# xxxupeng/stereo_toolbox

Measured on AMD Instinct MI355X. Metric: stereo pairs/sec @ 540x960 D=192 (GwcNet_GC fwd+bwd), higher is better.
Workload: dtype f32; 1 GPU; GwcNet_GC(maxdisp=192) train step: fwd+bwd+allreduce+Adam, 576x960 pairs (reference pad_to_2x shape), batch 1/GPU, fp32, synthetic randn inputs, deterministic filler weights; global_batch=1, parallelism=dp1, grad_sync=none (single rank: flat fp32 buffer packed, no collective), launch=eager, optimizer=torch.optim.Adam(fused=True)

## Files before the change

stereo_toolbox_amd/csrc/conv3d.hip:

```cpp
#include "stx_common.h"
#include <stdlib.h>

namespace {

constexpr int CONV_THREADS = 256;

struct ConvArgs {
    const float* x;
    const float* wp;
    float* out;
    const float* scale;
    const float* bias;
    const float* residual;
    float* stats;
    int Di, Hi, Wi, Cin;
    int Do, Ho, Wo, Cout;
    int relu;
    int nDt, nHt, nWt;
};

__device__ __forceinline__ int xcd_remap(int bid, int nblk) {
    const int q = nblk >> 3, r = nblk & 7;
    const int xcd = bid & 7, k = bid >> 3;
    const int base = (xcd < r) ? xcd * (q + 1) : r * (q + 1) + (xcd - r) * q;
// ... 873 lines not shown
    const float* f;
    const float* c;
    float* slab;
    int B, Df, Hf, Wf, CF;
    int Dc, Hc, Wc, CC;
    int nHt, nWt, ntiles;
    int ablate;
};

template <int KS, int S, int TH, int TW, int NW, bool PIPE>
__global__ __launch_bounds__(NW * 64) void conv3d_wgrad_kernel(WgradArgs a) {
    constexpr int NTHR = NW * 64;
    constexpr int PAD = KS / 2;
    constexpr int T = KS * KS * KS;
    constexpr int ED = KS, EH = (TH - 1) * S + KS, EW = (TW - 1) * S + KS;
    constexpr int EWH = (EW + 1) / 2;
    constexpr int EWS = (S == 2) ? 2 * EWH : EW;
    constexpr int NTAP = (T + NW - 1) / NW;
    constexpr int NV = TH * TW;
    STX_DYN_SMEM(smem);
    float* ftile = reinterpret_cast<float*>(smem);
    float* ctile = ftile + ED * EH * EWS * 32;

    const int tid = threadIdx.x, lane = tid & 63;
    const int wave = __builtin_amdgcn_readfirstlane(tid >> 6);
    const int i = lane & 31, half = lane >> 5;
    const int ncf = a.CF / 32;
    const int cfb = blockIdx.y % ncf, ccb = blockIdx.y / ncf;

    f32x16 acc[NTAP];
#pragma unroll
    for (int t = 0; t < NTAP; ++t) acc[t] = zero16();

    constexpr int NPL = (EH * EW * 8 + NTHR - 1) / NTHR;
    constexpr int NFL = ED * NPL;
    constexpr int NCL = (NV * 8 + NTHR - 1) / NTHR;
    float4 sf[NFL], sc[NCL];
    unsigned fbase[NPL], cbase[NCL];
    int fhw[NPL], chw[NCL];
#pragma unroll
    for (int k = 0; k < NPL; ++k) {
        const int idx = tid + k * NTHR;
        const int v = idx >> 3, f = idx & 7;
        const int wx = v % EW, hy = v / EW;
        fhw[k] = idx < EH * EW * 8 ? (hy << 16 | wx) : -1;
        fbase[k] = (unsigned)(((hy * a.Wf + wx) * a.CF + cfb * 32 + 4 * f) * 4);
    }
#pragma unroll
    for (int k = 0; k < NCL; ++k) {
        const int idx = tid + k * NTHR;
        const int v = idx >> 3, f = idx & 7;
        chw[k] = idx < NV * 8 ? ((v / TW) << 16 | (v % TW)) : -1;
        cbase[k] = (unsigned)((((v / TW) * a.Wc + v % TW) * a.CC + ccb * 32 + 4 * f) * 4);
    }
    const long long fplane = (long long)a.Hf * a.Wf, cplane = (long long)a.Hc * a.Wc;
    auto load_tile = [&](int tile, bool on) {
        int r = tile;
        const int wt = r % a.nWt; r /= a.nWt;
        const int ht = r % a.nHt; r /= a.nHt;
        const int od = r % a.Dc;
        const int b = r / a.Dc;
        const int oh0 = ht * TH, ow0 = wt * TW;
        const int id0 = od * S - PAD, ih0 = oh0 * S - PAD, iw0 = ow0 * S - PAD;
        unsigned fvo[NPL];
#pragma unroll
        for (int k = 0; k < NPL; ++k) {
            const int gh = ih0 + (fhw[k] >> 16), gw = iw0 + (fhw[k] & 0xffff);
            fvo[k] = (fhw[k] >= 0 && gh >= 0 && gh < a.Hf && gw >= 0 && gw < a.Wf) ? fbase[k] : STX_BUF_OOB;
        }
        const long long forg = (long long)ih0 * a.Wf + iw0;
#pragma unroll
        for (int dz = 0; dz < ED; ++dz) {
            const int gd = id0 + dz;
            const bool in = on && gd >= 0 && gd < a.Df;
            const stx_bufrsrc rs = stx_make_rsrc(a.f + (((long long)b * a.Df + (in ? gd : 0)) * fplane + forg) * a.CF,
                                                 in ? (unsigned)((fplane - forg) * a.CF * 4) : 0u);
#pragma unroll
            for (int k = 0; k < NPL; ++k) sf[dz * NPL + k] = stx_buf_ld4(rs, fvo[k], 0u);
        }
        const long long corg = (long long)oh0 * a.Wc + ow0;
        const stx_bufrsrc rc = stx_make_rsrc(a.c + (((long long)b * a.Dc + od) * cplane + corg) * a.CC,
                                             on ? (unsigned)((cplane - corg) * a.CC * 4) : 0u);
#pragma unroll
        for (int k = 0; k < NCL; ++k) {
            const bool ok = chw[k] >= 0 && oh0 + (chw[k] >> 16) < a.Hc && ow0 + (chw[k] & 0xffff) < a.Wc;
            sc[k] = stx_buf_ld4(rc, ok ? cbase[k] : STX_BUF_OOB, 0u);
        }
    };
    auto store_tile = [&]() {
#pragma unroll
        for (int dz = 0; dz < ED; ++dz)
#pragma unroll
            for (int k = 0; k < NPL; ++k) {
                const int wx = fhw[k] & 0xffff, hy = fhw[k] >> 16;
                const int slot = (S == 2) ? (wx & 1) * EWH + (wx >> 1) : wx;
                const int f = (tid + k * NTHR) & 7;
                if (fhw[k] >= 0) stx_st4(ftile + ((dz * EH + hy) * EWS + slot) * 32 + 4 * f, sf[dz * NPL + k]);
            }
#pragma unroll
        for (int k = 0; k < NCL; ++k) {
            const int idx = tid + k * NTHR;
            if (idx < NV * 8) stx_st4(ctile + (idx >> 3) * 32 + 4 * (idx & 7), sc[k]);
        }
    };

    if (PIPE && (int)blockIdx.x < a.ntiles) load_tile(blockIdx.x, a.ablate != 1);
    for (int tile = blockIdx.x; tile < a.ntiles; tile += gridDim.x) {
        if (!PIPE) load_tile(tile, a.ablate != 1);
        __syncthreads();
        if (a.ablate != 1) store_tile();
        __syncthreads();
        if (PIPE) {
            const int nxt = tile + (int)gridDim.x;
            load_tile(nxt < a.ntiles ? nxt : tile, nxt < a.ntiles && a.ablate != 1);
        }
        if (a.ablate == 2) continue;
        if (KS == 1) {
            for (int p = wave; p < NV / 2; p += NW) {
                const int v = 2 * p + half;
                const int lw = v % TW, lh = v / TW;
                const float bv = ctile[v * 32 + i];
                const float av = ftile[(lh * EWS + lw) * 32 + i];
                acc[0] = __builtin_amdgcn_mfma_f32_32x32x2f32(av, bv, acc[0], 0, 0, 0);
            }
        } else {
            int toff[NTAP];
#pragma unroll
            for (int t = 0; t < NTAP; ++t) {
                const int tap = (t * NW + wave < T) ? t * NW + wave : 0;
                const int kd = tap / 9, kh = (tap / 3) % 3, kw = tap % 3;
                toff[t] = (S == 2) ? ((kd * EH + kh) * EWS + (kw & 1) * EWH + (kw >> 1)) * 32
                                   : ((kd * EH + kh) * EWS + kw) * 32;
            }
            float av[2][NTAP], bv[2];
            auto load_pair = [&](int p, int buf) {
                const int v = 2 * p + half;
                const int lw = v % TW, lh = v / TW;
                const int vb = ((lh * S) * EWS + lw) * 32 + i;
                bv[buf] = ctile[v * 32 + i];
#pragma unroll
                for (int t = 0; t < NTAP; ++t) av[buf][t] = ftile[vb + toff[t]];
            };
            auto mma_pair = [&](int buf) {
#pragma unroll
                for (int t = 0; t < NTAP; ++t)
                    if (t * NW + wave < T) acc[t] = __builtin_amdgcn_mfma_f32_32x32x2f32(av[buf][t], bv[buf], acc[t], 0, 0, 0);
            };
            load_pair(0, 0);
            for (int p = 0; p < NV / 2; p += 2) {
                load_pair(p + 1, 1);
                STX_SCHED_BARRIER();
                mma_pair(0);
                STX_SCHED_BARRIER();
                load_pair((p + 2 < NV / 2) ? p + 2 : 0, 0);
                STX_SCHED_BARRIER();
                mma_pair(1);
                STX_SCHED_BARRIER();
            }
        }
    }
    constexpr int ROWS = (KS == 1) ? NW : T;
    float* dst = a.slab + ((size_t)blockIdx.y * gridDim.x + blockIdx.x) * ROWS * 1024;
#pragma unroll
    for (int t = 0; t < NTAP; ++t) {
        const int row = (KS == 1) ? wave : t * NW + wave;
        if (KS == 1 ? (t == 0) : (row < T)) {
#pragma unroll
            for (int r = 0; r < 16; ++r) {
                const int cf = (r & 3) + 8 * (r >> 2) + 4 * half;
                dst[(size_t)row * 1024 + cf * 32 + i] = acc[t][r];
            }
        }
    }
}

__global__ __launch_bounds__(CONV_THREADS) void conv3d_wgrad_reduce4_kernel(const float* __restrict__ slab,
                                                                            float* __restrict__ dw, int CF, int CC,
                                                                            int T, int nchunks, int rows_per_chunk) {
    __shared__ float red[16][64];
    const int lane = threadIdx.x & 63, wave = threadIdx.x >> 6;
    const int part = wave * 4 + (lane >> 4), ql = lane & 15;
    const int idx0 = blockIdx.x * 64 + ql * 4;
    const int cc_l = idx0 & 31, cf_l = (idx0 >> 5) & 31;
    const int tap = (idx0 >> 10) % T, pair = (idx0 >> 10) / T;
    const float* p;
    size_t stride;
    int n;
    if (rows_per_chunk == T) {
        p = slab + ((size_t)pair * nchunks * T + tap) * 1024 + cf_l * 32 + cc_l;
        stride = (size_t)T * 1024; n = nchunks;
    } else {
        p = slab + ((size_t)pair * nchunks * rows_per_chunk) * 1024 + cf_l * 32 + cc_l;
        stride = 1024; n = nchunks * rows_per_chunk;
    }
    float4 s = make_float4(0.f, 0.f, 0.f, 0.f);
#pragma unroll 4
    for (int c = part; c < n; c += 16) {
        const float4 v = stx_ld4(p + (size_t)c * stride);
        s.x += v.x; s.y += v.y; s.z += v.z; s.w += v.w;
    }
    stx_st4(&red[part][ql * 4], s);
    __syncthreads();
    if (wave == 0) {
        float t = 0.f;
#pragma unroll
        for (int k = 0; k < 16; ++k) t += red[k][lane];
        const int idx = blockIdx.x * 64 + lane;
        const int cc = idx & 31, cf = (idx >> 5) & 31;
        const int ncf = CF / 32, cfb = pair % ncf, ccb = pair / ncf;
        dw[((size_t)(ccb * 32 + cc) * CF + cfb * 32 + cf) * T + tap] = t;
    }
}

template <typename K, typename... Args>
int launch_with_lds(K kernel, dim3 grid, size_t lds, hipStream_t st, Args... args) {
    if (int rc = stx_lds_require((const void*)kernel, lds, "conv3d")) return rc;
    static const bool report = getenv("STX_REPORT_OCCUPANCY") != nullptr;
    if (report) {
        int nb = -1;
        hipOccupancyMaxActiveBlocksPerMultiprocessor(&nb, (const void*)kernel, CONV_THREADS, lds);
        fprintf(stderr, "[stx] conv3d launch: grid %u x %u, %zu B LDS, %d workgroups per CU\n", grid.x, grid.y, lds, nb);
    }
    hipLaunchKernelGGL(kernel, grid, dim3(CONV_THREADS), lds, st, args...);
    return 0;
}

constexpr int CONV_TD = 2, CONV_TH = 2;

template <int KS, int S>
size_t conv_lds_bytes(int CK, int NT) {
    const int ED = (CONV_TD - 1) * S + KS, EH = (CONV_TH - 1) * S + KS, EW = 31 * S + KS;
    const int EWS = (S == 2) ? 2 * ((EW + 1) / 2) : EW;
    size_t t = (size_t)ED * EH * EWS * (CK + 4) * 4;
    size_t red = (size_t)4 * NT * 32 * 2 * 4;
    return t > red ? t : red;
}

template <int S>
void (*pgemm_kernel(int wn))(ConvArgs, int) {
    return wn == 4 ? conv3d_pgemm_kernel<3, S, CONV_TD, CONV_TH, 4, 8, 4>
         : wn == 2 ? conv3d_pgemm_kernel<3, S, CONV_TD, CONV_TH, 4, 8, 2> : conv3d_pgemm_kernel<3, S, CONV_TD, CONV_TH, 4, 8>;
}

void (*march_kernel(int bs, int epi))(MarchArgs) {
    switch (epi) {
    case 0: return bs ? conv3d_marchw_kernel<1, 0> : conv3d_marchw_kernel<0, 0>;
    case 2: return bs ? conv3d_marchw_kernel<1, 2> : conv3d_marchw_kernel<0, 2>;
    case 3: return bs ? conv3d_marchw_kernel<1, 3> : conv3d_marchw_kernel<0, 3>;
    case 4: return bs ? conv3d_marchw_kernel<1, 4> : conv3d_marchw_kernel<0, 4>;
    case 5: return bs ? conv3d_marchw_kernel<1, 5> : conv3d_marchw_kernel<0, 5>;
    default: return bs ? conv3d_marchw_kernel<1, 1> : conv3d_marchw_kernel<0, 1>;
    }
}

template <int KS, int S>
int conv_dispatch(const ConvArgs& a, int NT, int CK, dim3 grid, hipStream_t st) {
    const size_t lds = conv_lds_bytes<KS, S>(CK, NT);
#define CONV_CASE(NT_, CK_)                                                                                        \
    if (NT == NT_ && CK == CK_)                                                                                    \
        return launch_with_lds(conv3d_igemm_kernel<KS, S, CONV_TD, CONV_TH, NT_, CK_>, grid, lds, st, a);
    if constexpr (KS == 1) { CONV_CASE(1, 32) CONV_CASE(2, 32) CONV_CASE(4, 32) }
    if constexpr (KS == 3) {
        if (NT == 2 && CK == 8 && stx_tune(STX_TUNE_CONV_WN) >= 2)
            return launch_with_lds(conv3d_igemm_kernel<KS, S, CONV_TD, CONV_TH, 2, 8, 4, 2>, grid, lds, st, a);
    }
    CONV_CASE(1, 8) CONV_CASE(2, 8) CONV_CASE(4, 8)
#undef CONV_CASE
    return stx_set_error(STX_ERR_ARG, "conv3d: unsupported NT=%d CK=%d", NT, CK);
}

}

static int conv_pick_ck(int Cin, int ks) { return (ks == 1 && Cin % 32 == 0) ? 32 : 8; }
static int conv_nt(int N) { return N <= 32 ? 1 : (N <= 64 ? 2 : 4); }

extern "C" long long stx_conv3d_packed_floats(int K, int N, int T) {
    return (long long)T * (K / 8) * conv_nt(N) * 256;
}

extern "C" int stx_conv3d_pack_weight(const float* w, float* wp, int A, int Bd, int T, int mode, void* stream) {
    stx_begin();
    STX_REQUIRE(w && wp && A > 0 && Bd > 0 && (T == 1 || T == 27), "conv3d_pack_weight: bad args");
    STX_REQUIRE(mode >= 0 && mode <= 2, "conv3d_pack_weight: mode %d", mode);
    const int K = (mode == 0) ? Bd : A, N = (mode == 0) ? A : Bd;
    STX_REQUIRE(K % 8 == 0 && N <= 128, "conv3d_pack_weight: GEMM-K channels (%d) must be a multiple of 8, N (%d) <= 128", K, N);
    const int NT = conv_nt(N);
    const size_t total = (size_t)T * (K / 8) * NT * 256;
    hipLaunchKernelGGL(conv3d_pack_kernel, dim3((unsigned)((total + CONV_THREADS - 1) / CONV_THREADS)),
                       dim3(CONV_THREADS), 0, (hipStream_t)stream, w, wp, A, Bd, T, mode, K, N, NT, total);
    return stx_check_launch("conv3d_pack_weight");
}

static int march_wgs(long long units) {
    long long g = 256;
    if (g > units / 3) g = units / 3;
    return g < 1 ? 1 : (int)g;
}

extern "C" int stx_conv3d_fwd_blocks(int Do, int Ho, int Wo) {
    stx_begin();
    const int a = stx_cdiv(Do, CONV_TD) * stx_cdiv(Ho, CONV_TH) * stx_cdiv(Wo, 32);
    const int m = Do * stx_cdiv(Ho, 4) * stx_cdiv(Wo, 32);
    const int m16 = Do * stx_cdiv(Ho, 8) * stx_cdiv(Wo, 16);
    return a > m ? (a > m16 ? a : m16) : (m > m16 ? m : m16);
}
extern "C" int stx_deconv3d_fwd_blocks(int Di, int Hi, int Wi) {
    stx_begin(); return Di * stx_cdiv(Hi, 2) * stx_cdiv(Wi, 32); }

struct ConvPlan { int kind; int march_wgs; int pgrid; long long rows; };
static int persistent_grid(size_t lds, long long ntiles) {
    int per_cu = (int)(STX_LDS_MAX / (lds + 512));
    per_cu = per_cu < 1 ? 1 : (per_cu > 2 ? 2 : per_cu);
    const long long g = 256ll * per_cu;
    return (int)(g > ntiles ? ntiles : g);
}
static ConvPlan conv_plan(int B, int Di, int Hi, int Wi, int Cin, int Cout, int ks, int stride) {
    const int pad = ks / 2;
    const int Do = (Di + 2 * pad - ks) / stride + 1, Ho = (Hi + 2 * pad - ks) / stride + 1, Wo = (Wi + 2 * pad - ks) / stride + 1;
    ConvPlan p{2, 0, 0, 0};
    if (ks == 3 && stride == 1 && ((Cin == 32 && Cout <= 64) || (Cin == 64 && Cout <= 32) ||
                                   (Cin == 64 && Cout <= 64 && stx_tune(STX_TUNE_CONV_L1_MARCH)))) {
        const long long ncols = (long long)B * stx_cdiv(Ho, MW2_TH) * stx_cdiv(Wo, MW2_MW);
        if (ncols * Do < (1ll << 31) && (long long)Hi * Wi * Cin * 4 < (1ll << 31) && (long long)Ho * Wo * Cout * 4 < (1ll << 31)) {
            p.kind = 0; p.march_wgs = march_wgs(ncols * Do); p.rows = p.march_wgs;
            return p;
        }
    }
    const long long tiles = (long long)stx_cdiv(Do, CONV_TD) * stx_cdiv(Ho, CONV_TH) * stx_cdiv(Wo, 32);
    if (conv_nt(Cout) == 4 && ks == 3 && tiles * B < (1ll << 31)) {
        const size_t lds = stride == 1 ? conv_lds_bytes<3, 1>(8, 4) : conv_lds_bytes<3, 2>(8, 4);
        p.kind = 1; p.pgrid = persistent_grid(lds, tiles * B); p.rows = p.pgrid;
        return p;
    }
    p.rows = tiles * B;
    return p;
}

extern "C" long long stx_conv3d_fwd_stat_rows(int B, int Di, int Hi, int Wi, int Cin, int Cout, int ks, int stride) {
    stx_begin();
    if (B < 1 || Di < 1 || Hi < 1 || Wi < 1 || Cin < 1 || Cout < 1 || !((ks == 3 && (stride == 1 || stride == 2)) || (ks == 1 && stride == 1)))
        return 0;
    return conv_plan(B, Di, Hi, Wi, Cin, Cout, ks, stride).rows;
}

extern "C" int stx_conv3d_fwd(const float* x, const float* wp, float* out, const float* scale, const float* bias,
                              const float* residual, float* stats, int B, int Di, int Hi, int Wi, int Cin, int Cout,
                              int ks, int stride, int relu, void* stream) {
    stx_begin();
    STX_REQUIRE(x && wp && out && B > 0 && Di > 0 && Hi > 0 && Wi > 0, "conv3d_fwd: bad shape");
    STX_REQUIRE(Cin % 8 == 0 && Cout >= 1 && Cout <= 128, "conv3d_fwd: Cin=%d (need %%8) Cout=%d (need <=128)", Cin, Cout);
    STX_REQUIRE((ks == 3 && (stride == 1 || stride == 2)) || (ks == 1 && stride == 1),
                "conv3d_fwd: kernel %d stride %d unsupported", ks, stride);
    ConvArgs a;
    a.x = x; a.wp = wp; a.out = out; a.scale = scale; a.bias = bias; a.residual = residual; a.stats = stats;
    a.Di = Di; a.Hi = Hi; a.Wi = Wi; a.Cin = Cin; a.Cout = Cout; a.relu = relu;
    const int pad = ks / 2;
    a.Do = (Di + 2 * pad - ks) / stride + 1;
    a.Ho = (Hi + 2 * pad - ks) / stride + 1;
    a.Wo = (Wi + 2 * pad - ks) / stride + 1;
    a.nDt = stx_cdiv(a.Do, CONV_TD); a.nHt = stx_cdiv(a.Ho, CONV_TH); a.nWt = stx_cdiv(a.Wo, 32);
    const int NT = conv_nt(Cout);
    hipStream_t st = (hipStream_t)stream;
    const ConvPlan plan = conv_plan(B, Di, Hi, Wi, Cin, Cout, ks, stride);
    if (plan.kind == 0) {
        MarchArgs m2;
        m2.c = a;
        m2.c.nHt = stx_cdiv(a.Ho, MW2_TH);
        m2.c.nWt = stx_cdiv(a.Wo, MW2_MW);
        m2.ncols = B * m2.c.nHt * m2.c.nWt;
        m2.ablate = stx_tune(STX_TUNE_MARCH_ABLATE);
        {
            const int nb2 = plan.march_wgs;
            const size_t lds2 = ((size_t)MW2_WFLOATS + 2 * (size_t)MW2_SLOT) * 4;
            const int bs = stx_tune(STX_TUNE_MARCH_BS), epi_fast = stx_tune(STX_TUNE_MARCH_EPI);
            const bool whole = a.Ho % MW2_TH == 0 && a.Wo % MW2_MW == 0;
            m2.xs = Cin; m2.os = Cout; m2.wq_total = Cin / 8; m2.wnt_total = conv_nt(Cout);
            const int nk = Cin / 32, nn = stx_cdiv(Cout, 32);
            for (int ns = 0; ns < nn; ++ns)
                for (int kslice = 0; kslice < nk; ++kslice) {
                    MarchArgs m = m2;
                    m.xo = 32 * kslice; m.wq_off = 4 * kslice;
                    m.oo = 32 * ns; m.wnt_off = ns; m.ncout = Cout - 32 * ns < 32 ? Cout - 32 * ns : 32;
                    m.acc_in = kslice > 0 ? out : nullptr;
                    if (kslice + 1 < nk) {
                        m.c.scale = nullptr; m.c.bias = nullptr; m.c.residual = nullptr; m.c.stats = nullptr; m.c.relu = 0;
                    }
                    const bool plain = epi_fast && !(m.c.residual && m.acc_in) && m.c.relu < 2;
                    const bool raw = !m.acc_in && !m.c.residual && !m.c.scale && !m.c.bias && m.c.relu == 0;
                    const int epi = plain ? (raw ? (whole && m.ncout == 32 ? 5 : 4) : m.acc_in ? 2 : (m.c.residual ? 3 : 0)) : 1;
                    if (int rc = launch_with_lds(march_kernel(bs, epi), dim3(nb2), lds2, st, m)) return rc;
                }
            return stx_check_launch("conv3d_fwd(march)");
        }
    }
    STX_REQUIRE(halo_range_ok(Di, Hi, Wi, Cin), "conv3d_fwd: a batch item of %d x %d x %d x %d floats exceeds the 2 GiB "
                "buffer-descriptor range", Di, Hi, Wi, Cin);
    const int CK = (stride == 2) ? 8 : conv_pick_ck(Cin, ks);
    dim3 grid(a.nDt * a.nHt * a.nWt, B);
    int rc;
    if (plan.kind == 1) {
        const long long nt_all = (long long)grid.x * B;
        {
            const size_t lds = stride == 1 ? conv_lds_bytes<3, 1>(8, 4) : conv_lds_bytes<3, 2>(8, 4);
            const int wn = stx_tune(STX_TUNE_CONV_WN) == 4 ? 4 : (stx_tune(STX_TUNE_CONV_WN) == 3 ? 2 : 1);
            rc = launch_with_lds(stride == 1 ? pgemm_kernel<1>(wn) : pgemm_kernel<2>(wn), dim3(plan.pgrid), lds, st, a, (int)nt_all);
            if (rc) return rc;
            return stx_check_launch("conv3d_fwd(pipelined)");
        }
    }
    if (ks == 3 && stride == 1) rc = conv_dispatch<3, 1>(a, NT, CK, grid, st);
    else if (ks == 3 && NT == 2 && stx_tune(STX_TUNE_CONV_S2_DENSE)) {
        if (stx_tune(STX_TUNE_CONV_WN) >= 2)
            rc = launch_with_lds(conv3d_igemm_kernel<3, 2, CONV_TD, CONV_TH, 2, 8, 0, 2>, grid, (size_t)5 * 5 * 66 * 8 * 4, st, a);
        else
        rc = launch_with_lds(conv3d_igemm_kernel<3, 2, CONV_TD, CONV_TH, 2, 8, 0>, grid, (size_t)5 * 5 * 66 * 8 * 4, st, a);
    }
    else if (ks == 3) rc = conv_dispatch<3, 2>(a, NT, CK, grid, st);
    else rc = conv_dispatch<1, 1>(a, NT, CK, grid, st);
    if (rc) return rc;
    return stx_check_launch("conv3d_fwd");
}

extern "C" int stx_deconv3d_fwd(const float* x, const float* wp, float* out, const float* scale, const float* bias,
                                const float* residual, float* stats, int B, int Di, int Hi, int Wi, int Cin, int Cout,
                                int Do, int Ho, int Wo, int relu, void* stream) {
    stx_begin();
    STX_REQUIRE(x && wp && out && B > 0 && Di > 0 && Hi > 0 && Wi > 0, "deconv3d_fwd: bad shape");
    STX_REQUIRE(Cin % 32 == 0 && Cout >= 1 && Cout <= 64, "deconv3d_fwd: Cin=%d (need %%32) Cout=%d (need <=64)", Cin, Cout);
    STX_REQUIRE(Do <= 2 * Di && Do >= 2 * Di - 1 && Ho <= 2 * Hi && Ho >= 2 * Hi - 1 && Wo <= 2 * Wi && Wo >= 2 * Wi - 1,
                "deconv3d_fwd: output dims must be 2*in or 2*in-1");
    ConvArgs a;
    a.x = x; a.wp = wp; a.out = out; a.scale = scale; a.bias = bias; a.residual = residual; a.stats = stats;
    a.Di = Di; a.Hi = Hi; a.Wi = Wi; a.Cin = Cin; a.Cout = Cout; a.relu = relu;
    a.Do = Do; a.Ho = Ho; a.Wo = Wo;
    a.nDt = Di; a.nHt = stx_cdiv(Hi, 2); a.nWt = stx_cdiv(Wi, 32);
    STX_REQUIRE(halo_range_ok(Di, Hi, Wi, Cin), "deconv3d_fwd: a batch item of %d x %d x %d x %d floats exceeds the 2 GiB "
                "buffer-descriptor range", Di, Hi, Wi, Cin);
    dim3 grid(a.nDt * a.nHt * a.nWt, B);
    hipStream_t st = (hipStream_t)stream;
    const size_t lds = (size_t)2 * 3 * 33 * (8 + 4) * 4;
    int rc = conv_nt(Cout) == 1 ? launch_with_lds(deconv3d_igemm_kernel<1, 8>, grid, lds, st, a)
                                : launch_with_lds(deconv3d_igemm_kernel<2, 8>, grid, lds, st, a);
    if (rc) return rc;
    return stx_check_launch("deconv3d_fwd");
}

static bool wgrad_pipe(int ks, int stride, int npairs) { return ks == 3 && (stride == 2 || npairs <= 2); }
static void wgrad_tile(int ks, int stride, int Wc, bool pipe, int* TH, int* TW) {
    *TH = pipe ? 4 : 2; *TW = (stride == 2) ? 16 : 32;
    if (ks == 3 && stride == 1 && stx_cdiv(Wc, 16) * 16 < stx_cdiv(Wc, 32) * 32) { *TH = 4; *TW = 16; }
}
static int wgrad_chunks(int ntiles, int npairs, bool pipe) {
    int c = (pipe ? 256 : 512) / npairs;
    if (c < 1) c = 1;
    if (c > ntiles) c = ntiles;
    const int forced = stx_tune(STX_TUNE_WGRAD_GRID);
    if (forced > 0 && forced < c) c = forced;
    return c;
}

struct StxWgradBn {
    const float* z; float* dz;
    const float *scale, *shift, *mean, *invstd, *gamma, *sum_g, *sum_gx;
    float inv_n; int act;
};
int stx_wgrad_march_launch(const float* x, const float* gy, float* slab, int B, int D, int H, int W, int CF, int CC, int nchunks,
                           void* stream, const StxWgradBn* bn);
int stx_wgrad_march_chunks(int B, int D, int H, int W, int npairs);
int stx_wgrad_march_s2_launch(const float* f, const float* c, float* slab, int B, int Df, int Hf, int Wf, int CF, int Dc, int Hc,
                              int Wc, int CC, int nchunks, void* stream);

extern "C" long long stx_conv3d_wgrad_workspace_floats(int B, int Dc, int Hc, int Wc, int CF, int CC, int ks,
                                                       int stride) {
    const int npairs = (CF / 32) * (CC / 32);
    if (npairs < 1 || B < 1 || Dc < 1 || Hc < 1 || Wc < 1) return 0;
    const int rows = (ks == 1) ? 8 : 27;
    const bool pipe = wgrad_pipe(ks, stride, npairs);
    int TH, TW;
    wgrad_tile(ks, stride, Wc, pipe, &TH, &TW);
    int c = wgrad_chunks(B * Dc * stx_cdiv(Hc, TH) * stx_cdiv(Wc, TW), npairs, pipe);
    if (ks == 3) {
        const int cm = stx_wgrad_march_chunks(B, Dc, Hc, Wc, npairs);
        if (cm > c) c = cm;
    }
    return (long long)npairs * c * rows * 1024;
}

extern "C" int stx_conv3d_wgrad(const float* f, const float* c, float* dw, float* workspace, int B, int Df, int Hf,
                                int Wf, int CF, int Dc, int Hc, int Wc, int CC, int ks, int stride, void* stream) {
    stx_begin();
    STX_REQUIRE(f && c && dw && workspace && B > 0, "conv3d_wgrad: null operand");
    STX_REQUIRE(CF >= 32 && CC >= 32 && CF % 32 == 0 && CC % 32 == 0,
                "conv3d_wgrad: channel counts (%d, %d) must be positive multiples of 32", CF, CC);
    STX_REQUIRE(Dc > 0 && Hc > 0 && Wc > 0, "conv3d_wgrad: empty volume");
    STX_REQUIRE((ks == 3 && (stride == 1 || stride == 2)) || (ks == 1 && stride == 1), "conv3d_wgrad: ks/stride");
    STX_REQUIRE((long long)Hf * Wf * CF * 4 < (1ll << 31) && (long long)Hc * Wc * CC * 4 < (1ll << 31),
                "conv3d_wgrad: a plane of %d x %d voxels exceeds the 2 GiB buffer-descriptor range", Hf, Wf);
    WgradArgs a;
    a.f = f; a.c = c; a.slab = workspace;
    a.B = B; a.Df = Df; a.Hf = Hf; a.Wf = Wf; a.CF = CF; a.Dc = Dc; a.Hc = Hc; a.Wc = Wc; a.CC = CC;
    const int npairs = (CF / 32) * (CC / 32);
    const bool pipe = wgrad_pipe(ks, stride, npairs);
    a.ablate = stx_tune(STX_TUNE_WGRAD_ABLATE);
    int TH, TW;
    wgrad_tile(ks, stride, Wc, pipe, &TH, &TW);
    a.nHt = stx_cdiv(Hc, TH); a.nWt = stx_cdiv(Wc, TW);
    a.ntiles = B * Dc * a.nHt * a.nWt;
    int nchunks = wgrad_chunks(a.ntiles, npairs, pipe);
    hipStream_t st = (hipStream_t)stream;
    const int T = ks == 1 ? 1 : 27;
    if (ks == 3 && (stx_tune(STX_TUNE_WGRAD_MARCH) & (stride == 1 ? 1 : 2))) {
        int mc = stx_wgrad_march_chunks(B, Dc, Hc, Wc, npairs);
        const int forced = stx_tune(STX_TUNE_WGRAD_GRID);
        if (forced > 0 && forced < mc) mc = forced;
        const int rc = stride == 1 ? stx_wgrad_march_launch(f, c, workspace, B, Dc, Hc, Wc, CF, CC, mc, stream, nullptr)
                                   : stx_wgrad_march_s2_launch(f, c, workspace, B, Df, Hf, Wf, CF, Dc, Hc, Wc, CC, mc, stream);
        if (rc > 0) return rc;
        if (rc == 0) {
            const int total = npairs * T * 1024;
            hipLaunchKernelGGL(conv3d_wgrad_reduce4_kernel, dim3(total / 64), dim3(CONV_THREADS), 0, st, workspace, dw, CF, CC, T,
                               mc, 27);
            return stx_check_launch("conv3d_wgrad_reduce");
        }
    }
    dim3 grid(nchunks, npairs);
#define WG_LAUNCH(KS_, S_, TH_, TW_, NW_, PIPE_, LDS_)                                                           \
    {                                                                                                             \
        const size_t lds = (LDS_);                                                                                \
        void (*wk)(WgradArgs) = conv3d_wgrad_kernel<KS_, S_, TH_, TW_, NW_, PIPE_>;                               \
        if (int rc = stx_lds_require((const void*)wk, lds, "conv3d_wgrad")) return rc;                            \
        hipLaunchKernelGGL(wk, grid, dim3(NW_ * 64), lds, st, a);                                                 \
    }
    if (ks == 3 && stride == 1) {
        if (TW == 16 && pipe) WG_LAUNCH(3, 1, 4, 16, 8, true, ((size_t)3 * 6 * 18 + 64) * 32 * 4)
        else if (TW == 16) WG_LAUNCH(3, 1, 4, 16, 8, false, ((size_t)3 * 6 * 18 + 64) * 32 * 4)
        else if (pipe) WG_LAUNCH(3, 1, 4, 32, 8, true, ((size_t)3 * 6 * 34 + 128) * 32 * 4)
        else WG_LAUNCH(3, 1, 2, 32, 8, false, ((size_t)3 * 4 * 34 + 64) * 32 * 4)
    } else if (ks == 3) {
        WG_LAUNCH(3, 2, 4, 16, 8, true, ((size_t)3 * 9 * 34 + 64) * 32 * 4)
    } else {
        WG_LAUNCH(1, 1, 2, 32, 4, false, ((size_t)2 * 32 + 64) * 32 * 4)
    }
#undef WG_LAUNCH
    int rc = stx_check_launch("conv3d_wgrad");
    if (rc) return rc;
    const int total = npairs * T * 1024;
    hipLaunchKernelGGL(conv3d_wgrad_reduce4_kernel, dim3(total / 64), dim3(CONV_THREADS), 0, st, workspace, dw, CF, CC, T,
                       nchunks, ks == 1 ? 4 : 27);
    return stx_check_launch("conv3d_wgrad_reduce");
}

extern "C" int stx_conv3d_wgrad_bn_supported(int B, int D, int H, int W, int CF, int CC) {
    stx_begin();
    return (stx_tune(STX_TUNE_WGRAD_MARCH) & 1) && B > 0 && D > 0 && H > 0 && W > 0 && CF >= 32 && CC >= 32 && CF % 32 == 0 &&
           CC % 32 == 0 && (long long)H * W * CF * 4 < (1ll << 31) && (long long)H * W * CC * 4 < (1ll << 31) &&
           (long long)B * stx_cdiv(H, 4) * stx_cdiv(W, 16) < (1ll << 31);
}

extern "C" int stx_conv3d_wgrad_bn(const float* x, const float* gy, const float* z, const float* scale, const float* shift,
                                   const float* mean, const float* invstd, const float* gamma, const float* sums, float inv_n,
                                   int act, float* dz, float* dw, float* workspace, int B, int D, int H, int W, int CF, int CC,
                                   void* stream) {
    stx_begin();
    STX_REQUIRE(x && gy && z && scale && shift && mean && invstd && sums && dz && dw && workspace, "conv3d_wgrad_bn: null operand");
    STX_REQUIRE(act == 0 || act == 1, "conv3d_wgrad_bn: activation code %d (0 or 1)", act);
    STX_REQUIRE(stx_conv3d_wgrad_bn_supported(B, D, H, W, CF, CC), "conv3d_wgrad_bn: shape (%d x %d x %d x %d, %d -> %d channels) is "
                "not served by the march kernel (ask stx_conv3d_wgrad_bn_supported)", B, D, H, W, CF, CC);
    const int npairs = (CF / 32) * (CC / 32);
    int mc = stx_wgrad_march_chunks(B, D, H, W, npairs);
    const int forced = stx_tune(STX_TUNE_WGRAD_GRID);
    if (forced > 0 && forced < mc) mc = forced;
    StxWgradBn bn;
    bn.z = z; bn.dz = dz; bn.scale = scale; bn.shift = shift; bn.mean = mean; bn.invstd = invstd; bn.gamma = gamma;
    bn.sum_g = sums; bn.sum_gx = sums + CC; bn.inv_n = inv_n; bn.act = act;
    const int rc = stx_wgrad_march_launch(x, gy, workspace, B, D, H, W, CF, CC, mc, stream, &bn);
    if (rc > 0) return rc;
    STX_REQUIRE(rc == 0, "conv3d_wgrad_bn: the march kernel refused the shape");
    const int total = npairs * 27 * 1024;
    hipLaunchKernelGGL(conv3d_wgrad_reduce4_kernel, dim3(total / 64), dim3(CONV_THREADS), 0, (hipStream_t)stream, workspace, dw, CF,
                       CC, 27, mc, 27);
    return stx_check_launch("conv3d_wgrad_reduce");
}
```

stereo_toolbox_amd/csrc/stx_common.h:

```cpp
#pragma once
#ifdef STX_HIPEMU
#include "hipemu.h"
#define STX_DYN_SMEM(name) char* name = hipemu::dyn_smem()
#define stx_exp(x) expf(x)
#define stx_fdiv(a, b) ((a) / (b))
#define STX_SCHED_BARRIER() ((void)0)
#define STX_SCHED_GROUP(mask, n) ((void)0)
#define STX_OPAQUE_VGPR(x) ((void)0)
#define STX_TIE3(a, b, c) ((void)0)
#define STX_BARRIER_LDS() __syncthreads()
#define STX_GLDS4(base, off, ldsptr) ((void)(((float*)(ldsptr))[threadIdx.x & 63u] = (base)[(off)]))
#define STX_GLDS_WAIT() ((void)0)
#else
#include <hip/hip_runtime.h>
#define STX_DYN_SMEM(name) extern __shared__ __attribute__((aligned(16))) char name[]
#ifdef STX_PRECISE_MATH
#define stx_exp(x) expf(x)
#define stx_fdiv(a, b) ((a) / (b))
#else
#define stx_exp(x) __expf(x)
#define stx_fdiv(a, b) __fdividef((a), (b))
#endif
#define STX_SCHED_BARRIER() __builtin_amdgcn_sched_barrier(0)
#define STX_SCHED_GROUP(mask, n) __builtin_amdgcn_sched_group_barrier(mask, n, 0)
#define STX_OPAQUE_VGPR(x) asm volatile("" : "+v"(x))
#define STX_TIE3(a, b, c) asm volatile("" : "+v"(a), "+v"(b), "+v"(c))
#define STX_BARRIER_LDS() asm volatile("s_waitcnt lgkmcnt(0)\n\ts_barrier" ::: "memory")
__device__ __forceinline__ void stx_glds4(const float* base, unsigned off, const float* ldsptr) {
    const unsigned dst = (unsigned)__builtin_amdgcn_readfirstlane(
        (int)(unsigned)(size_t)(const __attribute__((address_space(3))) void*)ldsptr);
    const unsigned boff = off * 4u;
    unsigned keep;
    asm volatile("s_mov_b32 %0, m0\n\ts_mov_b32 m0, %3\n\ts_nop 0\n\tglobal_load_lds_dword %1, %2\n\ts_mov_b32 m0, %0"
                 : "=&s"(keep)
                 : "v"(boff), "s"(base), "s"(dst)
                 : "memory");
}
#define STX_GLDS4(base, off, ldsptr) stx_glds4((base), (off), (ldsptr))
#define STX_GLDS_WAIT() asm volatile("s_waitcnt vmcnt(0)" ::: "memory")
#endif
#define STX_BUF_OOB 0x80000000u
#ifdef STX_HIPEMU
struct stx_bufrsrc { const char* base; unsigned bytes; };
static inline stx_bufrsrc stx_make_rsrc(const void* p, unsigned bytes) { return stx_bufrsrc{(const char*)p, bytes}; }
static inline float4 stx_buf_ld4(stx_bufrsrc r, unsigned voff, unsigned soff) {
    const unsigned long long off = (unsigned long long)voff + soff;
    if (voff >= STX_BUF_OOB || off + 16 > r.bytes) return make_float4(0.f, 0.f, 0.f, 0.f);
    return *reinterpret_cast<const float4*>(r.base + off);
}
static inline float stx_buf_ld1(stx_bufrsrc r, unsigned voff, unsigned soff) {
    const unsigned long long off = (unsigned long long)voff + soff;
    if (voff >= STX_BUF_OOB || off + 4 > r.bytes) return 0.f;
    return *reinterpret_cast<const float*>(r.base + off);
}
static inline void stx_buf_st1(stx_bufrsrc r, unsigned voff, unsigned soff, float v) {
    if (voff >= STX_BUF_OOB || voff >= r.bytes) return;
    const unsigned long long off = (unsigned long long)voff + soff;
    if (off + 4 > r.bytes) abort();
    *reinterpret_cast<float*>(const_cast<char*>(r.base) + off) = v;
}
static inline void stx_buf_st4(stx_bufrsrc r, unsigned voff, unsigned soff, float4 v) {
    if (voff >= STX_BUF_OOB || voff >= r.bytes) return;
    const unsigned long long off = (unsigned long long)voff + soff;
    if (off + 16 > r.bytes) abort();
    *reinterpret_cast<float4*>(const_cast<char*>(r.base) + off) = v;
}
#else
typedef __amdgpu_buffer_rsrc_t stx_bufrsrc;
typedef unsigned int stx_u32x4 __attribute__((ext_vector_type(4)));
__device__ __forceinline__ stx_bufrsrc stx_make_rsrc(const void* p, unsigned bytes) {
    return __builtin_amdgcn_make_buffer_rsrc(const_cast<void*>(p), 0, (int)bytes, 0x00020000);
}
__device__ __forceinline__ float4 stx_buf_ld4(stx_bufrsrc r, unsigned voff, unsigned soff) {
    const stx_u32x4 v = __builtin_amdgcn_raw_buffer_load_b128(r, (int)voff, (int)soff, 0);
    return make_float4(__uint_as_float(v[0]), __uint_as_float(v[1]), __uint_as_float(v[2]), __uint_as_float(v[3]));
}
__device__ __forceinline__ float stx_buf_ld1(stx_bufrsrc r, unsigned voff, unsigned soff) {
    return __uint_as_float(__builtin_amdgcn_raw_buffer_load_b32(r, (int)voff, (int)soff, 0));
}
__device__ __forceinline__ void stx_buf_st1(stx_bufrsrc r, unsigned voff, unsigned soff, float v) {
    __builtin_amdgcn_raw_buffer_store_b32(__float_as_uint(v), r, (int)voff, (int)soff, 0);
}
__device__ __forceinline__ void stx_buf_st4(stx_bufrsrc r, unsigned voff, unsigned soff, float4 v) {
    const stx_u32x4 u = {__float_as_uint(v.x), __float_as_uint(v.y), __float_as_uint(v.z), __float_as_uint(v.w)};
    __builtin_amdgcn_raw_buffer_store_b128(u, r, (int)voff, (int)soff, 0);
}
#endif
template <typename T>
__device__ __forceinline__ T* stx_uniform_ptr(T* p) {
    const unsigned long long v = (unsigned long long)p;
    const unsigned lo = (unsigned)__builtin_amdgcn_readfirstlane((int)(unsigned)v);
    const unsigned hi = (unsigned)__builtin_amdgcn_readfirstlane((int)(unsigned)(v >> 32));
    return (T*)(((unsigned long long)hi << 32) | lo);
}
#include <stdint.h>

typedef float f32x4 __attribute__((ext_vector_type(4)));
typedef float f32x16 __attribute__((ext_vector_type(16)));

#define STX_OK 0
#define STX_ERR_ARG 1
#define STX_ERR_LAUNCH 2

int stx_set_error(int code, const char* fmt, ...);
int stx_check_launch(const char* what);
static inline void stx_begin() { (void)hipGetLastError(); }

#define STX_REQUIRE(cond, ...)                                   \
    do {                                                         \
        if (!(cond)) return stx_set_error(STX_ERR_ARG, __VA_ARGS__); \
    } while (0)

static inline int stx_cdiv(int a, int b) { return (a + b - 1) / b; }

constexpr size_t STX_LDS_DEFAULT = 64 * 1024;
constexpr size_t STX_LDS_MAX = 160 * 1024;
bool stx_lds_try(const void* kern, size_t bytes);
int stx_lds_require(const void* kern, size_t bytes, const char* what);

enum StxTune {
    STX_TUNE_MARCH_BS,
    STX_TUNE_MARCH_EPI,
    STX_TUNE_MARCH_ABLATE,
    STX_TUNE_WGRAD_ABLATE,
    STX_TUNE_WGRAD_MARCH,
    STX_TUNE_WGRAD_GRID,
    STX_TUNE_CONV_L1_MARCH,
    STX_TUNE_CONV_S2_DENSE,
    STX_TUNE_CONV_WN,
    STX_TUNE_CV_OLD,
    STX_TUNE_CV_GRID,
    STX_TUNE_CV_PF,
    STX_TUNE_CV_UNITS,
    STX_TUNE_CV_WIN,
    STX_TUNE_CVB_OLD,
    STX_TUNE_CVB_TEAM,
    STX_TUNE_CVB_GRID,
    STX_TUNE_CVB_NSET,
    STX_TUNE_SV_BWD_V1,
    STX_TUNE_DWCONV_ROLL,
    STX_TUNE_C2_PAD,
    STX_TUNE_C2_ABLATE,
    STX_TUNE_COUNT
};
int stx_tune(StxTune id);

__device__ __forceinline__ float stx_mish_tanh_sp(float x, float& w) {
    w = stx_exp(x < 20.f ? x : 20.f);
    const float n = w * (w + 2.f);
    return x > 20.f ? 1.f : stx_fdiv(n, n + 2.f);
}
__device__ __forceinline__ float stx_mish(float x) {
    float w;
    return x * stx_mish_tanh_sp(x, w);
}
__device__ __forceinline__ float stx_mish_grad(float x) {
    float w;
    const float t = stx_mish_tanh_sp(x, w);
    const float ds = x > 20.f ? 1.f : stx_fdiv(w, 1.f + w);
    return t + x * (1.f - t * t) * ds;
}
#define STX_LEAKY_SLOPE 0.01f
__device__ __forceinline__ float stx_act(float v, int code) {
    return code == 1 ? (v > 0.f ? v : 0.f) : (code == 2 ? stx_mish(v) : (code == 3 ? (v > 0.f ? v : STX_LEAKY_SLOPE * v) : v));
}
__device__ __forceinline__ float stx_act_bwd(float g, float t, int code) {
    return code == 2 ? g * stx_mish_grad(t) : (code == 3 ? (t > 0.f ? g : STX_LEAKY_SLOPE * g) : (t > 0.f ? g : 0.f));
}

__device__ __forceinline__ float4 stx_ld4(const float* p) { return *reinterpret_cast<const float4*>(p); }
__device__ __forceinline__ void stx_st4(float* p, float4 v) { *reinterpret_cast<float4*>(p) = v; }
__device__ __forceinline__ void stx_st4_nt(float* p, float4 v) {
#ifdef STX_HIPEMU
    *reinterpret_cast<float4*>(p) = v;
#else
    f32x4 t;
    t[0] = v.x; t[1] = v.y; t[2] = v.z; t[3] = v.w;
    __builtin_nontemporal_store(t, reinterpret_cast<f32x4*>(p));
#endif
}
```

stereo_toolbox_amd/csrc/stx_runtime.hip:

```cpp
#include "stx_common.h"
#include <stdarg.h>
#include <stdio.h>

static thread_local char g_err[512] = "";

int stx_set_error(int code, const char* fmt, ...) {
    va_list ap;
    va_start(ap, fmt);
    vsnprintf(g_err, sizeof(g_err), fmt, ap);
    va_end(ap);
    return code;
}

int stx_check_launch(const char* what) {
    hipError_t e = hipGetLastError();
    if (e != hipSuccess) return stx_set_error(STX_ERR_LAUNCH, "%s: launch failed: %s", what, hipGetErrorString(e));
    return STX_OK;
}

bool stx_lds_try(const void* kern, size_t bytes) {
    if (bytes <= STX_LDS_DEFAULT) return true;
    if (bytes > STX_LDS_MAX) return false;
    if (hipFuncSetAttribute(kern, hipFuncAttributeMaxDynamicSharedMemorySize, (int)bytes) == hipSuccess) return true;
    (void)hipGetLastError();
    return false;
}

int stx_lds_require(const void* kern, size_t bytes, const char* what) {
    if (bytes > STX_LDS_MAX) return stx_set_error(STX_ERR_ARG, "%s: %zu B of LDS exceed the %zu B of a CU", what, bytes, STX_LDS_MAX);
    if (!stx_lds_try(kern, bytes)) return stx_set_error(STX_ERR_LAUNCH, "%s: %zu B of LDS refused by this device", what, bytes);
    return STX_OK;
}

extern "C" const char* stx_last_error(void) { return g_err; }

extern "C" const char* stx_build_info(void) {
#ifdef STX_HIPEMU
    return "stx-hipemu (host SIMT emulator build: tests only)";
#else
    return "stx-gfx950 (hipcc --offload-arch=gfx950)";
#endif
}

#include <stdlib.h>
#include <string.h>
namespace {
struct TuneEntry { const char* name; int value; };
TuneEntry g_tune[STX_TUNE_COUNT] = {
    {"STX_MARCH_BS", 1}, {"STX_MARCH_EPI", 1}, {"STX_MARCH_ABLATE", 0}, {"STX_WGRAD_ABLATE", 0}, {"STX_WGRAD_MARCH", 3}, {"STX_WGRAD_GRID", 0}, {"STX_CONV_L1_MARCH", 0}, {"STX_CONV_S2_DENSE", 1}, {"STX_CONV_WN", 2},
    {"STX_CV_OLD", 0}, {"STX_CV_GRID", 0}, {"STX_CV_PF", 0}, {"STX_CV_UNITS", 1}, {"STX_CV_WIN", 0}, {"STX_CVB_OLD", 0}, {"STX_CVB_TEAM", 0}, {"STX_CVB_GRID", 0}, {"STX_CVB_NSET", 3},
    {"STX_SV_BWD_V1", 0}, {"STX_DWCONV_ROLL", 1}, {"STX_C2_PAD", 8}, {"STX_C2_ABLATE", 0},
};
struct TuneInit {
    TuneInit() {
        for (int i = 0; i < STX_TUNE_COUNT; ++i)
            if (const char* e = getenv(g_tune[i].name)) g_tune[i].value = atoi(e);
    }
} g_tune_init;
}

int stx_tune(StxTune id) { return g_tune[id].value; }

extern "C" int stx_get_tuning(const char* name) {
    for (int i = 0; i < STX_TUNE_COUNT; ++i)
        if (name && !strcmp(name, g_tune[i].name)) return g_tune[i].value;
    return -1;
}

extern "C" int stx_set_tuning(const char* name, int value) {
    for (int i = 0; i < STX_TUNE_COUNT; ++i)
        if (name && !strcmp(name, g_tune[i].name)) { g_tune[i].value = value; return STX_OK; }
    return stx_set_error(STX_ERR_ARG, "stx_set_tuning: unknown switch %s", name ? name : "(null)");
}
```

Baseline: 0.1785 pairs/s.

## Add depth-marching kernel for stride-2 3D conv 32->64 channels

Adds a dedicated kernel for the stride-2, 3x3x3, 32-to-64-channel 3D convolution. Each workgroup keeps all weights for one 32-channel output slice resident in LDS and marches along depth over a fixed set of output columns. Each input plane is loaded once and reused by up to two output depths through split partial accumulators, and BN statistics are emitted per run. This targets the redundant halo and weight reloads of the generic tiled path. In exchange it uses a fixed grid of about 128 runs, which may underfill the GPU. It applies only without a fused scale, bias, residual or ReLU epilogue; with an epilogue it falls back and requires that no stats be requested.

```diff
diff --git a/stereo_toolbox_amd/csrc/conv3d.hip b/stereo_toolbox_amd/csrc/conv3d.hip
--- a/stereo_toolbox_amd/csrc/conv3d.hip
+++ b/stereo_toolbox_amd/csrc/conv3d.hip
@@ -1199,12 +1199,17 @@
     const int a = stx_cdiv(Do, CONV_TD) * stx_cdiv(Ho, CONV_TH) * stx_cdiv(Wo, 32);
     const int m = Do * stx_cdiv(Ho, 4) * stx_cdiv(Wo, 32);
     const int m16 = Do * stx_cdiv(Ho, 8) * stx_cdiv(Wo, 16);
-    return a > m ? (a > m16 ? a : m16) : (m > m16 ? m : m16);
+    const int m8 = Do * stx_cdiv(Ho, 8) * stx_cdiv(Wo, 8);
+    const int am = a > m ? a : m, mm = m16 > m8 ? m16 : m8;
+    return am > mm ? am : mm;
 }
 extern "C" int stx_deconv3d_fwd_blocks(int Di, int Hi, int Wi) {
     stx_begin(); return Di * stx_cdiv(Hi, 2) * stx_cdiv(Wi, 32); }
 
 struct ConvPlan { int kind; int march_wgs; int pgrid; long long rows; };
+int stx_conv3d_s2_march_runs(int B, int Di, int Hi, int Wi, int Cin, int Cout);
+int stx_conv3d_s2_march_launch(const float* x, const float* wp, float* out, float* stats, int B, int Di, int Hi, int Wi,
+                               int nruns, hipStream_t st);
 static int persistent_grid(size_t lds, long long ntiles) {
     int per_cu = (int)(STX_LDS_MAX / (lds + 512));
     per_cu = per_cu < 1 ? 1 : (per_cu > 2 ? 2 : per_cu);
@@ -1220,6 +1225,12 @@
         const long long ncols = (long long)B * stx_cdiv(Ho, MW2_TH) * stx_cdiv(Wo, MW2_MW);
         if (ncols * Do < (1ll << 31) && (long long)Hi * Wi * Cin * 4 < (1ll << 31) && (long long)Ho * Wo * Cout * 4 < (1ll << 31)) {
             p.kind = 0; p.march_wgs = march_wgs(ncols * Do); p.rows = p.march_wgs;
+            return p;
+        }
+    }
+    if (ks == 3 && stride == 2) {
+        if (const int runs = stx_conv3d_s2_march_runs(B, Di, Hi, Wi, Cin, Cout)) {
+            p.kind = 3; p.march_wgs = runs; p.rows = runs;
             return p;
         }
     }
@@ -1290,6 +1301,11 @@
             return stx_check_launch("conv3d_fwd(march)");
         }
     }
+    if (plan.kind == 3) {
+        if (!scale && !bias && !residual && relu == 0)
+            return stx_conv3d_s2_march_launch(x, wp, out, stats, B, Di, Hi, Wi, plan.march_wgs, st);
+        STX_REQUIRE(!stats, "conv3d_fwd: stride-2 32 -> 64 with an epilogue writes no statistics rows (STX_CONV_S2_MARCH=0 does)");
+    }
     STX_REQUIRE(halo_range_ok(Di, Hi, Wi, Cin), "conv3d_fwd: a batch item of %d x %d x %d x %d floats exceeds the 2 GiB "
                 "buffer-descriptor range", Di, Hi, Wi, Cin);
     const int CK = (stride == 2) ? 8 : conv_pick_ck(Cin, ks);
diff --git a/stereo_toolbox_amd/csrc/conv3d_s2_march.hip b/stereo_toolbox_amd/csrc/conv3d_s2_march.hip
--- /dev/null
+++ b/stereo_toolbox_amd/csrc/conv3d_s2_march.hip
@@ -0,0 +1,242 @@
+#include "stx_common.h"
+
+namespace {
+
+constexpr int S2M_THREADS = 256;
+constexpr int S2M_T = 8;
+constexpr int S2M_E = 2 * S2M_T + 1;
+constexpr int S2M_EWH = S2M_T + 1;
+constexpr int S2M_EWS = 20, S2M_VS = 36;
+constexpr int S2M_PLANE = S2M_E * S2M_EWS * S2M_VS;
+constexpr int S2M_WFLOATS = 27 * 1024;
+constexpr int S2M_NF4 = (S2M_E * S2M_E * 8 + S2M_THREADS - 1) / S2M_THREADS;
+constexpr size_t S2M_LDS = ((size_t)S2M_WFLOATS + S2M_PLANE) * 4;
+static_assert((2 * S2M_EWS * S2M_VS) % 64 == 32 && S2M_VS % 64 == 36, "conflict-free operand reads");
+static_assert(S2M_LDS <= STX_LDS_MAX, "LDS");
+
+struct S2mArgs {
+    const float* x;
+    const float* wp;
+    float* out;
+    float* stats;
+    int Di, Hi, Wi, Do, Ho, Wo;
+    int nHt, nWt, ncols;
+    int nruns;
+};
+
+typedef float f32x4v __attribute__((ext_vector_type(4)));
+__device__ __forceinline__ f32x4v s2m_zero() { f32x4v z = {0.f, 0.f, 0.f, 0.f}; return z; }
+
+__global__ __launch_bounds__(S2M_THREADS) void conv3d_s2_march_kernel(S2mArgs a) {
+    constexpr int CIN = 32, COUT = 64;
+    STX_DYN_SMEM(smem);
+    float* wl = reinterpret_cast<float*>(smem);
+    float* plane = wl + S2M_WFLOATS;
+    const int tid = threadIdx.x, lane = tid & 63, wave = __builtin_amdgcn_readfirstlane(tid >> 6);
+    const int i = lane & 15, kq = lane >> 4;
+    const int grp = blockIdx.x >> 4, rem = blockIdx.x & 15;
+    const int run = __builtin_amdgcn_readfirstlane(grp * 8 + (rem & 7)), slice = __builtin_amdgcn_readfirstlane(rem >> 3);
+    if (run >= a.nruns) return;
+
+    for (int e = tid; e < S2M_WFLOATS / 4; e += S2M_THREADS) {
+        const int l = e & 63, nb = (e >> 6) & 1, g = (e >> 7) & 1, tap = e >> 8;
+        const int n = l & 15, k4 = l >> 4;
+        const int q = 2 * g + (k4 >> 1), half = k4 & 1;
+        const size_t src = ((size_t)(tap * 4 + q) * 2 + slice) * 256 + (size_t)(half * 32 + 16 * nb + n) * 4;
+        stx_st4(wl + 4 * e, stx_ld4(a.wp + src));
+    }
+
+    const long long units = (long long)a.ncols * a.Do;
+    int u = __builtin_amdgcn_readfirstlane((int)(units * run / a.nruns));
+    const int u_end = __builtin_amdgcn_readfirstlane((int)(units * (run + 1) / a.nruns));
+
+    const unsigned xplane_bytes = (unsigned)a.Hi * (unsigned)a.Wi * CIN * 4u;
+    const unsigned oplane_bytes = (unsigned)a.Ho * (unsigned)a.Wo * COUT * 4u;
+    int b = 0, oh0 = 0, ow0 = 0;
+    float4 stg[S2M_NF4];
+    unsigned svoff[S2M_NF4], ovoff[4];
+    auto column_offsets = [&]() {
+#pragma unroll
+        for (int k = 0; k < S2M_NF4; ++k) {
+            const int e = tid + k * S2M_THREADS;
+            const int v = e >> 3, f = e & 7;
+            const int wy = v / S2M_E, wx = v - wy * S2M_E;
+            const int gh = 2 * oh0 - 1 + wy, gw = 2 * ow0 - 1 + wx;
+            const bool ok = v < S2M_E * S2M_E && gh >= 0 && gh < a.Hi && gw >= 0 && gw < a.Wi;
+            svoff[k] = ok ? (unsigned)(((gh * a.Wi + gw) * CIN + 4 * f) * 4) : STX_BUF_OOB;
+        }
+        const int oh = oh0 + 2 * wave + (kq >> 1), owb = ow0 + 4 * (kq & 1);
+#pragma unroll
+        for (int r = 0; r < 4; ++r)
+            ovoff[r] = (oh < a.Ho && owb + r < a.Wo) ? (unsigned)((((oh * a.Wo + owb + r) * COUT) + 32 * slice + i) * 4) : STX_BUF_OOB;
+    };
+    auto load_plane = [&](int p) {
+        const bool in = p >= 0 && p < a.Di;
+        const stx_bufrsrc rs = stx_make_rsrc(a.x + ((size_t)b * a.Di + (in ? p : 0)) * a.Hi * a.Wi * CIN, in ? xplane_bytes : 0u);
+#pragma unroll
+        for (int k = 0; k < S2M_NF4; ++k) stg[k] = stx_buf_ld4(rs, svoff[k], 0u);
+    };
+    auto store_plane = [&]() {
+#pragma unroll
+        for (int k = 0; k < S2M_NF4; ++k) {
+            const int e = tid + k * S2M_THREADS;
+            const int v = e >> 3, f = e & 7;
+            const int wy = v / S2M_E, wx = v - wy * S2M_E;
+            const int slot = (wx & 1) * S2M_EWH + (wx >> 1);
+            if (v < S2M_E * S2M_E) stx_st4(plane + (wy * S2M_EWS + slot) * S2M_VS + 4 * f, stg[k]);
+        }
+    };
+
+    const int abase = ((2 * (2 * wave + (i >> 3))) * S2M_EWS + (i & 7)) * S2M_VS + 4 * kq;
+    const float* wlane = wl + lane * 4;
+
+    auto tap_plane = [&](int kd, f32x4v (&acc)[2]) {
+        float4 av[2][2], bv[2][2][2];
+        auto load_tap = [&](int t9, int buf) {
+            const int kh = t9 / 3, kw = t9 % 3;
+            const float* sl = plane + abase + (kh * S2M_EWS + (kw == 1 ? S2M_EWH : (kw >> 1))) * S2M_VS;
+            const float* wt = wlane + (kd * 9 + t9) * 1024;
+#pragma unroll
+            for (int g = 0; g < 2; ++g) {
+                av[buf][g] = stx_ld4(sl + 16 * g);
+                bv[buf][g][0] = stx_ld4(wt + (2 * g) * 256);
+                bv[buf][g][1] = stx_ld4(wt + (2 * g + 1) * 256);
+            }
+        };
+        load_tap(0, 0);
+#pragma unroll
+        for (int t9 = 0; t9 < 9; ++t9) {
+            if (t9 + 1 < 9) load_tap(t9 + 1, (t9 + 1) & 1);
+            const int cb = t9 & 1;
+#pragma unroll
+            for (int g = 0; g < 2; ++g) {
+                acc[0] = __builtin_amdgcn_mfma_f32_16x16x4f32(av[cb][g].x, bv[cb][g][0].x, acc[0], 0, 0, 0);
+                acc[1] = __builtin_amdgcn_mfma_f32_16x16x4f32(av[cb][g].x, bv[cb][g][1].x, acc[1], 0, 0, 0);
+                acc[0] = __builtin_amdgcn_mfma_f32_16x16x4f32(av[cb][g].y, bv[cb][g][0].y, acc[0], 0, 0, 0);
+                acc[1] = __builtin_amdgcn_mfma_f32_16x16x4f32(av[cb][g].y, bv[cb][g][1].y, acc[1], 0, 0, 0);
+                acc[0] = __builtin_amdgcn_mfma_f32_16x16x4f32(av[cb][g].z, bv[cb][g][0].z, acc[0], 0, 0, 0);
+                acc[1] = __builtin_amdgcn_mfma_f32_16x16x4f32(av[cb][g].z, bv[cb][g][1].z, acc[1], 0, 0, 0);
+                acc[0] = __builtin_amdgcn_mfma_f32_16x16x4f32(av[cb][g].w, bv[cb][g][0].w, acc[0], 0, 0, 0);
+                acc[1] = __builtin_amdgcn_mfma_f32_16x16x4f32(av[cb][g].w, bv[cb][g][1].w, acc[1], 0, 0, 0);
+            }
+            if (t9 + 1 < 9) {
+#pragma unroll
+                for (int s = 0; s < 6; ++s) {
+                    STX_SCHED_GROUP(0x008, 2);
+                    STX_SCHED_GROUP(0x100, 1);
+                }
+            }
+            STX_SCHED_BARRIER();
+        }
+    };
+
+    float s1[2] = {0.f, 0.f}, s2[2] = {0.f, 0.f};
+    auto emit = [&](int od, const f32x4v (&c0)[2], const f32x4v (&c1)[2], const f32x4v (&c2)[2]) {
+        const stx_bufrsrc ors = stx_make_rsrc(a.out + ((size_t)b * a.Do + od) * a.Ho * a.Wo * COUT, oplane_bytes);
+#pragma unroll
+        for (int nb = 0; nb < 2; ++nb)
+#pragma unroll
+            for (int r = 0; r < 4; ++r) {
+                float v = (c0[nb][r] + c1[nb][r]) + c2[nb][r];
+                v = ovoff[r] != STX_BUF_OOB ? v : 0.f;
+                s1[nb] += v;
+                s2[nb] = fmaf(v, v, s2[nb]);
+                stx_buf_st1(ors, ovoff[r], (unsigned)(16 * nb * 4), v);
+            }
+    };
+
+    __syncthreads();
+    while (u < u_end) {
+        int d_lo, d_hi;
+        {
+            const int col = u / a.Do;
+            d_lo = u - col * a.Do;
+            const int left = u_end - u;
+            d_hi = (a.Do - d_lo < left) ? a.Do : d_lo + left;
+            u += d_hi - d_lo;
+            const int wt = col % a.nWt, ht = (col / a.nWt) % a.nHt;
+            b = col / (a.nWt * a.nHt);
+            oh0 = ht * S2M_T; ow0 = wt * S2M_T;
+        }
+        column_offsets();
+        const int p_lo = 2 * d_lo - 1, p_hi = 2 * d_hi - 1;
+        f32x4v c0[2], c1[2], c2[2], n0[2];
+#pragma unroll
+        for (int nb = 0; nb < 2; ++nb) c0[nb] = c1[nb] = c2[nb] = n0[nb] = s2m_zero();
+        load_plane(p_lo);
+        for (int p = p_lo; p <= p_hi; ++p) {
+            const bool live = p >= 0 && p < a.Di;
+            __syncthreads();
+            store_plane();
+            __syncthreads();
+            if (p < p_hi) load_plane(p + 1);
+            if (p & 1) {
+                const int od = (p - 1) >> 1;
+                const bool fin = od >= d_lo, start = od + 1 < d_hi;
+#pragma unroll
+                for (int nb = 0; nb < 2; ++nb) { c2[nb] = s2m_zero(); n0[nb] = s2m_zero(); }
+                if (live && fin) tap_plane(2, c2);
+                if (live && start) tap_plane(0, n0);
+                if (fin) emit(od, c0, c1, c2);
+#pragma unroll
+                for (int nb = 0; nb < 2; ++nb) c0[nb] = n0[nb];
+            } else {
+#pragma unroll
+                for (int nb = 0; nb < 2; ++nb) c1[nb] = s2m_zero();
+                if (live) tap_plane(1, c1);
+            }
+        }
+    }
+    if (a.stats) {
+#pragma unroll
+        for (int nb = 0; nb < 2; ++nb) {
+            s1[nb] += __shfl_xor(s1[nb], 16); s1[nb] += __shfl_xor(s1[nb], 32);
+            s2[nb] += __shfl_xor(s2[nb], 16); s2[nb] += __shfl_xor(s2[nb], 32);
+        }
+        __syncthreads();
+        if (lane < 16) {
+#pragma unroll
+            for (int nb = 0; nb < 2; ++nb) {
+                plane[(wave * 32 + 16 * nb + lane) * 2 + 0] = s1[nb];
+                plane[(wave * 32 + 16 * nb + lane) * 2 + 1] = s2[nb];
+            }
+        }
+        __syncthreads();
+        if (tid < 32) {
+            float t1 = 0.f, t2 = 0.f;
+#pragma unroll
+            for (int w = 0; w < 4; ++w) {
+                t1 += plane[(w * 32 + tid) * 2 + 0];
+                t2 += plane[(w * 32 + tid) * 2 + 1];
+            }
+            a.stats[(size_t)run * 2 * COUT + 32 * slice + tid] = t1;
+            a.stats[(size_t)run * 2 * COUT + COUT + 32 * slice + tid] = t2;
+        }
+    }
+}
+
+}
+
+int stx_conv3d_s2_march_runs(int B, int Di, int Hi, int Wi, int Cin, int Cout) {
+    if (!stx_tune(STX_TUNE_CONV_S2_MARCH) || Cin != 32 || Cout != 64) return 0;
+    const int Do = (Di - 1) / 2 + 1, Ho = (Hi - 1) / 2 + 1, Wo = (Wi - 1) / 2 + 1;
+    const long long units = (long long)B * stx_cdiv(Ho, S2M_T) * stx_cdiv(Wo, S2M_T) * Do;
+    if (units >= (1ll << 31) || (long long)Hi * Wi * Cin * 4 >= (1ll << 31) || (long long)Ho * Wo * Cout * 4 >= (1ll << 31)) return 0;
+    if (!stx_lds_try((const void*)conv3d_s2_march_kernel, S2M_LDS)) return 0;
+    const int forced = stx_tune(STX_TUNE_CONV_S2_GRID);
+    const long long r = forced > 0 ? forced : 128;
+    return (int)(r < units ? r : units);
+}
+
+int stx_conv3d_s2_march_launch(const float* x, const float* wp, float* out, float* stats, int B, int Di, int Hi, int Wi,
+                               int nruns, hipStream_t st) {
+    S2mArgs a;
+    a.x = x; a.wp = wp; a.out = out; a.stats = stats;
+    a.Di = Di; a.Hi = Hi; a.Wi = Wi;
+    a.Do = (Di - 1) / 2 + 1; a.Ho = (Hi - 1) / 2 + 1; a.Wo = (Wi - 1) / 2 + 1;
+    a.nHt = stx_cdiv(a.Ho, S2M_T); a.nWt = stx_cdiv(a.Wo, S2M_T); a.ncols = B * a.nHt * a.nWt;
+    a.nruns = nruns;
+    if (int rc = stx_lds_require((const void*)conv3d_s2_march_kernel, S2M_LDS, "conv3d_s2_march")) return rc;
+    hipLaunchKernelGGL(conv3d_s2_march_kernel, dim3(16 * stx_cdiv(nruns, 8)), dim3(S2M_THREADS), S2M_LDS, st, a);
+    return stx_check_launch("conv3d_fwd(s2 march)");
+}
diff --git a/stereo_toolbox_amd/csrc/stx_common.h b/stereo_toolbox_amd/csrc/stx_common.h
--- a/stereo_toolbox_amd/csrc/stx_common.h
+++ b/stereo_toolbox_amd/csrc/stx_common.h
@@ -127,6 +127,8 @@
     STX_TUNE_WGRAD_GRID,
     STX_TUNE_CONV_L1_MARCH,
     STX_TUNE_CONV_S2_DENSE,
+    STX_TUNE_CONV_S2_MARCH,
+    STX_TUNE_CONV_S2_GRID,
     STX_TUNE_CONV_WN,
     STX_TUNE_CV_OLD,
     STX_TUNE_CV_GRID,
diff --git a/stereo_toolbox_amd/csrc/stx_runtime.hip b/stereo_toolbox_amd/csrc/stx_runtime.hip
--- a/stereo_toolbox_amd/csrc/stx_runtime.hip
+++ b/stereo_toolbox_amd/csrc/stx_runtime.hip
@@ -47,7 +47,7 @@
 namespace {
 struct TuneEntry { const char* name; int value; };
 TuneEntry g_tune[STX_TUNE_COUNT] = {
-    {"STX_MARCH_BS", 1}, {"STX_MARCH_EPI", 1}, {"STX_MARCH_ABLATE", 0}, {"STX_WGRAD_ABLATE", 0}, {"STX_WGRAD_MARCH", 3}, {"STX_WGRAD_GRID", 0}, {"STX_CONV_L1_MARCH", 0}, {"STX_CONV_S2_DENSE", 1}, {"STX_CONV_WN", 2},
+    {"STX_MARCH_BS", 1}, {"STX_MARCH_EPI", 1}, {"STX_MARCH_ABLATE", 0}, {"STX_WGRAD_ABLATE", 0}, {"STX_WGRAD_MARCH", 3}, {"STX_WGRAD_GRID", 0}, {"STX_CONV_L1_MARCH", 0}, {"STX_CONV_S2_DENSE", 1}, {"STX_CONV_S2_MARCH", 1}, {"STX_CONV_S2_GRID", 0}, {"STX_CONV_WN", 2},
     {"STX_CV_OLD", 0}, {"STX_CV_GRID", 0}, {"STX_CV_PF", 0}, {"STX_CV_UNITS", 1}, {"STX_CV_WIN", 0}, {"STX_CVB_OLD", 0}, {"STX_CVB_TEAM", 0}, {"STX_CVB_GRID", 0}, {"STX_CVB_NSET", 3},
     {"STX_SV_BWD_V1", 0}, {"STX_DWCONV_ROLL", 1}, {"STX_C2_PAD", 8}, {"STX_C2_ABLATE", 0},
 };
```

New measurement: 0.1788 pairs/s, median of 2. No clear change (+0.2%).
